# leerob/pixo

Measured on NVIDIA H100. Metric: Mpixels/sec JPEG q=80 4:2:0 encode of 3840x2160 RGB, higher is better.
Workload: dtype f32

## Files before the change

### pixo_b200/csrc/api.cu

```cuda
#include <stdarg.h>
#include <stdlib.h>
#include <string.h>

#include <emmintrin.h>

#include <algorithm>
#include <cmath>
#include <thread>
#include <vector>

#include "common.cuh"
#include "jpeg_host.hpp"
#include "resize_host.hpp"

namespace pixo {

static thread_local std::string g_thread_err;

int set_error(pixo_b200_ctx *ctx, int code, const char *fmt, ...)
{
    char buf[512];
    va_list ap;
    va_start(ap, fmt);
    vsnprintf(buf, sizeof buf, fmt, ap);
// ... 404 lines not shown
    const uint8_t *vals[4];
    for (int k = 0; k < 4; ++k) {
        memcpy(bits[k], dht + k * 272, 16);
        vals[k] = dht + k * 272 + 16;
    }
    if (!prog_tables(bits, vals, T))
        return set_error(ctx, PIXO_B200_ERR_INVALID_ARGUMENT,
                         "Huffman table: more than 256 values, or a code that does not fit its length");
    return 0;
}

static int check_room(pixo_b200_ctx *ctx, size_t out_cap, size_t need)
{
    if (need > out_cap)
        return set_error(ctx, PIXO_B200_ERR_OUTPUT_TOO_SMALL, "output capacity %zu too small (need %zu)", out_cap, need);
    return 0;
}

static int finish_frame(pixo_b200_ctx *ctx, uint8_t *out, size_t out_cap, size_t hdr, size_t body, size_t *out_len)
{
    if (body == (size_t)-1)
        return set_error(ctx, PIXO_B200_ERR_OUTPUT_TOO_SMALL, "output capacity %zu too small", out_cap);
    PIXO_TRY(check_room(ctx, out_cap, hdr + body + 2));
    out[hdr + body] = 0xFF;
    out[hdr + body + 1] = 0xD9;
    *out_len = hdr + body + 2;
    return 0;
}

struct CoefLayout {
    size_t yb, cbb, yeb, ceb, each;
    explicit CoefLayout(const FrameGeometry &g)
        : yb(Layout::round(g.ny * 64 * sizeof(int16_t))), cbb(Layout::round(g.nc * 64 * sizeof(int16_t))),
          yeb(Layout::round(g.ny)), ceb(Layout::round(g.nc)), each(yb + 2 * cbb + yeb + 2 * ceb) {}
    size_t stride() const { return each / sizeof(int16_t); }
    int16_t *y(void *frame) const { return reinterpret_cast<int16_t *>(frame); }
    int16_t *cb(void *frame) const { return reinterpret_cast<int16_t *>(static_cast<uint8_t *>(frame) + yb); }
    int16_t *cr(void *frame) const { return reinterpret_cast<int16_t *>(static_cast<uint8_t *>(frame) + yb + cbb); }
    CoefExtents extents(void *frame) const
    {
        uint8_t *e = static_cast<uint8_t *>(frame) + yb + 2 * cbb;
        return CoefExtents{e, e + yeb, e + yeb + ceb, each};
    }
};

static void expand_records(const CoefLayout &L, const FrameGeometry &g, void *frame)
{
    const CoefExtents e = L.extents(frame);
    int16_t *arr[3] = {L.y(frame), L.cb(frame), L.cr(frame)};
    const uint8_t *ext[3] = {e.y, e.cb, e.cr};
    const size_t nb[3] = {g.ny, g.nc, g.nc};
    for (int c = 0; c < (g.has_chroma ? 3 : 1); ++c)
        for (size_t b = 0; b < nb[c]; ++b) {
            const int sectors = ext[c][b];
            memset(arr[c] + b * 64 + sectors * 16, 0, (size_t)(4 - sectors) * 32);
        }
}

void pixo_b200_quant_tables(int quality, uint8_t lum_zz[64], uint8_t chr_zz[64], float lum[64],
                            float chr[64])
{
    quant_tables(quality, lum_zz, chr_zz, lum, chr);
}

int pixo_b200_jpeg_block_counts(uint32_t width, uint32_t height, uint32_t color_type,
                                uint32_t subsampling, size_t *ny, size_t *nc)
{
    PIXO_TRY(validate_jpeg(nullptr, width, height, color_type, subsampling));
    const FrameGeometry g = make_geometry(width, height, color_type, subsampling);
    if (ny) *ny = g.ny;
    if (nc) *nc = g.nc;
    return 0;
}

static int trellis_status(pixo_b200_ctx *ctx, const uint32_t *d_status)
{
    PIXO_TRY(ctx->h_trellis.ensure(ctx, sizeof(uint32_t)));
    PIXO_CUDA(ctx, cudaMemcpyAsync(ctx->h_trellis.ptr, d_status, sizeof(uint32_t), cudaMemcpyDeviceToHost, ctx->stream));
    PIXO_CUDA(ctx, cudaStreamSynchronize(ctx->stream));
    if (*static_cast<const uint32_t *>(ctx->h_trellis.ptr))
        return set_error(ctx, PIXO_B200_ERR_INVALID_ARGUMENT,
                         "trellis input out of range: a non-finite value or cost, a non-zero |dct| below 2^-100, or |dct / q| above 32766");
    return 0;
}

static constexpr size_t kTrellisScratch = (size_t)256 << 20;

static int trellis_pieces(pixo_b200_ctx *ctx, const uint8_t *d_pixels, size_t pixel_stride, uint32_t n_images,
// ... 1478 lines not shown
```

### pixo_b200/csrc/common.cuh

```cuda
#pragma once

#include <cuda_runtime.h>
#include <stdint.h>
#include <stdio.h>

#include <atomic>
#include <condition_variable>
#include <functional>
#include <memory>
#include <mutex>
#include <string>
#include <thread>
#include <unordered_map>
#include <utility>
#include <vector>

#include "../../include/pixo_b200.h"

namespace pixo {

constexpr int kHistWords = 536;
constexpr size_t kDhtBytes = 4 * 272;
constexpr size_t kHuffDevBytes = 1632;

__host__ __device__ constexpr int zz_nat(int i)
{
    constexpr int t[64] = {0,  1,  8,  16, 9,  2,  3,  10, 17, 24, 32, 25, 18, 11, 4,  5,
                           12, 19, 26, 33, 40, 48, 41, 34, 27, 20, 13, 6,  7,  14, 21, 28,
                           35, 42, 49, 56, 57, 50, 43, 36, 29, 22, 15, 23, 30, 37, 44, 51,
                           58, 59, 52, 45, 38, 31, 39, 46, 53, 60, 61, 54, 47, 55, 62, 63};
    return t[i];
}

struct CoefExtents {
    uint8_t *y, *cb, *cr;
    size_t stride;
};

constexpr uint32_t kOvfNoFit = 1u;
constexpr uint32_t kOvfFault = 2u;
constexpr uint32_t kOvfSegment = 4u;
constexpr uint32_t kOvfRange = 8u;
constexpr uint32_t kOvfInput = 16u;

template <bool Pinned>
struct Buffer {
    void *ptr = nullptr;
    size_t cap = 0;
    Buffer() = default;
    Buffer(const Buffer &) = delete;
    Buffer &operator=(const Buffer &) = delete;
    ~Buffer()
    {
        if (ptr) Pinned ? cudaFreeHost(ptr) : cudaFree(ptr);
    }
    int ensure(pixo_b200_ctx *ctx, size_t bytes);
    uint8_t *slot(size_t i, size_t stride) const { return static_cast<uint8_t *>(ptr) + i * stride; }
};
using DevBuf = Buffer<false>;
using PinnedBuf = Buffer<true>;

class HostPool {
public:
    explicit HostPool(int nthreads);
    ~HostPool();
    void run(int njobs, const std::function<void(int)> &fn);

private:
    void worker();
    std::vector<std::thread> threads_;
// ... 233 lines not shown
```

### pixo_b200/csrc/jpeg_entropy.cu

```cuda
#include <type_traits>

#include "common.cuh"
#include "jpeg_host.hpp"

namespace pixo {
namespace {

constexpr int AC_STRIDE = 12, AC_ZRL = 190, AC_EOB = 191, AC_WORDS = 192;
struct HuffDev {
    uint32_t dc[2][12];
    uint32_t ac[2][AC_WORDS];
};
static_assert(sizeof(HuffDev) == kHuffDevBytes, "common.cuh sizes the per-frame tables by kHuffDevBytes");
struct HuffHalf {
    uint32_t dc[12];
    uint32_t ac[AC_WORDS];
};
struct FrameTables {
    const HuffDev *tabs;
};

struct EntParams {
    const int16_t *y, *cb, *cr;
    size_t y_stride, c_stride;
// ... 327 lines not shown
        uint32_t srel[NPASS], t7[NPASS];
#pragma unroll 1
        for (int p = 0; p < NPASS; ++p) {
            uint32_t mm, kk, comp;
            if (ypm == 4) {
                if (p < 2) { mm = 8 * p + (lane >> 2); kk = lane & 3; comp = 0; }
                else { mm = lane & 15; kk = 4 + (lane >> 4); comp = 1 + (lane >> 4); }
            } else if (bpm == 3) {
                mm = lane; kk = p; comp = p;
            } else {
                mm = 32 * p + lane; kk = 0; comp = 0;
            }
            const uint32_t sr = mm * bpm + kk;
            const bool valid = sr < nv;
            uint32_t *const slot = M.slot[p];
            uint32_t L = 0, tail7 = 0;
            int nwt = 0;
            if (__any_sync(0xffffffffu, valid)) {
                if constexpr (TABLES) {
                    const uint32_t half = comp ? 1u : 0u;
                    const uint32_t key = ((RAW && P.seg_per_img > 1) ? C.img / P.seg_per_img : C.img) * 2u + half;
                    if (key != tab_key) {
                        const uint32_t *src = reinterpret_cast<const uint32_t *>(Tp.tabs + (key >> 1));
                        uint32_t *dst = reinterpret_cast<uint32_t *>(&T[threadIdx.x >> 5]);
                        __syncwarp();
                        for (int i = lane; i < 12 + AC_WORDS; i += 32)
                            dst[i] = __ldg(src + (i < 12 ? half * 12 + i : 24 + half * AC_WORDS + (i - 12)));
                        __syncwarp();
                        tab_key = key;
                    }
                }
                const uint32_t m = mu0 + mm;
                const int16_t *arr;
                const uint8_t *earr;
                size_t idx, eidx;
                int seed;
                if (comp == 0) { arr = P.y + y_off; earr = P.e.y; idx = (size_t)m * ypm + kk; eidx = ey_off + idx; seed = P.dc_seed[0]; }
                else if (comp == 1) { arr = P.cb + c_off; earr = P.e.cb; idx = m; eidx = ec_off + idx; seed = P.dc_seed[1]; }
                else { arr = P.cr + c_off; earr = P.e.cr; idx = m; eidx = ec_off + idx; seed = P.dc_seed[2]; }
                const bool from_left = lane != 0 && !(ypm == 4 && p == 2 && lane == 16);
                int prev_ld = 0;
                if (valid && !from_left) {
                    const bool dc_reset = P.rst_mcus && C.first && mm == 0;
                    if (P.dc_seed_dev && idx == 0 && !seg_prev) seed = P.dc_seed_dev[comp];
                    prev_ld = dc_reset ? 0 : ((idx || seg_prev) ? arr[((long long)idx - 1) * 64] : seed);
                }
                int dc = 0;
                uint32_t M0 = 0, M1 = 0;
                if (valid) {
                    const uint4 *src = reinterpret_cast<const uint4 *>(arr + idx * 64);
                    uint32_t w[32];
                    if (CHECK) {
                        uint32_t n[32];
#pragma unroll
                        for (int q = 0; q < 8; ++q) {
                            const uint4 v = __ldg(src + q);
                            n[q * 4] = v.x; n[q * 4 + 1] = v.y; n[q * 4 + 2] = v.z; n[q * 4 + 3] = v.w;
                        }
                        dc = (int)(int16_t)(n[0] & 0xFFFF);
#pragma unroll
                        for (int j = 0; j < 32; ++j) {
                            const int i0 = zz_nat(2 * j), i1 = zz_nat(2 * j + 1);
                            w[j] = __byte_perm(n[i0 >> 1], n[i1 >> 1],
                                               ((i0 & 1) ? 0x0032 : 0x0010) | ((i1 & 1) ? 0x7600 : 0x5400));
                        }
#pragma unroll
                        for (int j = 0; j < 32; ++j) M.stage[j * CB + lane] = w[j];
                    } else {
                        const int np = 2 * __ldg(earr + eidx);
#pragma unroll
                        for (int q = 0; q < 8; ++q) {
                            const uint4 v = (q < 2 || q < np) ? __ldg(src + q) : make_uint4(0, 0, 0, 0);
                            w[q * 4] = v.x; w[q * 4 + 1] = v.y; w[q * 4 + 2] = v.z; w[q * 4 + 3] = v.w;
                        }
                        dc = (int)(int16_t)(w[0] & 0xFFFF);
#pragma unroll
                        for (int q = 0; q < 8; ++q) {
                            if (q < 2 || q < np) {
#pragma unroll
                                for (int t = 0; t < 4; ++t) M.stage[(q * 4 + t) * CB + lane] = w[q * 4 + t];
                            }
                        }
                    }
                    asm volatile("" ::: "memory");
                    {
                        uint32_t e0 = 0, e1 = 0;
#pragma unroll
                        for (int j = 0; j < 16; ++j) {
                            e0 += __vminu2(w[j], 0x00010001u) * (1u << j);
                            e1 += __vminu2(w[16 + j], 0x00010001u) * (1u << j);
                        }
                        M0 = interleave16(e0); M1 = interleave16(e1);
                    }
                }
                const int left = __shfl_up_sync(0xffffffffu, dc, 1);
                const int diff = (int)(int16_t)(dc - (from_left ? left : prev_ld));
                if (valid) {
                    const int tbl = comp ? 1 : 0;
                    const uint32_t *dctab;
                    uint32_t sa_ac;
                    if constexpr (TABLES) {
                        dctab = T[threadIdx.x >> 5].dc;
                        sa_ac = (uint32_t)__cvta_generic_to_shared(&T[threadIdx.x >> 5].ac[0]);
                    } else {
                        dctab = T.dc[tbl];
                        sa_ac = (uint32_t)__cvta_generic_to_shared(&T.ac[tbl][0]);
                    }
                    const uint32_t sa_slot = (uint32_t)__cvta_generic_to_shared(slot) + 4u * lane;
                    uint32_t acc;
                    bool bad;
                    L = code_block<false, CHECK>(M0, M1, diff, dctab, sa_ac, sa_stage, sa_slot, spill[p], &acc, &bad);
                    if (L > SLOT_W * 32u)
                        L = code_block<true, CHECK>(M0, M1, diff, dctab, sa_ac, sa_stage, sa_slot, spill[p], &acc, &bad);
                    if (CHECK && bad) atomicOr(&P.overflow[C.img], kOvfRange);
                    asm volatile("" ::: "memory");
                    const int nw = (int)(L >> 5), filled = (int)(L & 31u);
                    nwt = nw;
                    if (filled) {
                        if (nw < SLOT_W) slot[nw * CB + lane] = acc; else spill[p][nw - SLOT_W] = acc;
                        nwt = nw + 1;
                    }
                    const uint32_t lastw = nw == 0 ? 0u : (nw - 1 < SLOT_W ? slot[(nw - 1) * CB + lane] : spill[p][nw - 1 - SLOT_W]);
                    tail7 = __funnelshift_rc(acc, lastw, 32 - filled) & 0x7Fu;
                }
            }
// ... 1129 lines not shown
```

### pixo_b200/csrc/jpeg_transform.cu

```cuda
#include <cuda.h>
#include <string.h>

#include <algorithm>

#include "common.cuh"

namespace pixo {
namespace {

#define FADD(a, b) __fadd_rn((a), (b))
#define FSUB(a, b) __fsub_rn((a), (b))
#define FMUL(a, b) __fmul_rn((a), (b))

#define AAN_A1 0.70710678118654752440f
#define AAN_A2 0.5411961f
#define AAN_A3 0.70710678118654752440f
#define AAN_A4 1.3065629f
#define AAN_A5 0.38268343f
#define AAN_S0 0.3535534f
#define AAN_S1 0.2548978f
#define AAN_S2 0.2705981f
#define AAN_S3 0.3006724f
#define AAN_S4 0.3535534f
#define AAN_S5 0.4499881f
// ... 177 lines not shown
}

struct __align__(16) QPair {
    float nd_lo, nd_hi, r_lo, r_hi;
};

struct QPairTab {
    QPair t[2][32];
};


__device__ __forceinline__ void dct_rows_x2(f2 (&R)[4][8], f2 (&C)[8][4])
{
    constexpr float SK[8] = {AAN_S0, AAN_S1, AAN_S2, AAN_S3, AAN_S4, AAN_S5, AAN_S6, AAN_S7};
#pragma unroll
    for (int i = 0; i < 4; ++i) {
        f2 o[8];
        aan_1d_x2_core(R[i], o);
#pragma unroll
        for (int j = 0; j < 4; ++j) {
            float a0, a1, b0, b1;
            mulc(o[2 * j], SK[2 * j], a0, a1);
            mulc(o[2 * j + 1], SK[2 * j + 1], b0, b1);
            C[2 * i][j] = pk(a0, b0);
            C[2 * i + 1][j] = pk(a1, b1);
        }
    }
}

enum CoefOut { kNatural, kZigzag, kRecords, kDct };

template <int OUT, typename TabFn>
__device__ __forceinline__ void dct_cols_quant_store_x2(f2 (&C)[8][4], TabFn tab, uint4 *__restrict__ out,
                                                        const int swz, uint8_t *eout, float *dout, float dscale)
{
    constexpr bool ZIGZAG = OUT != kNatural;
    constexpr float SK[8] = {AAN_S0, AAN_S1, AAN_S2, AAN_S3, AAN_S4, AAN_S5, AAN_S6, AAN_S7};
    if constexpr (OUT == kDct) {
#pragma unroll
        for (int j = 0; j < 4; ++j) {
            const f2 in[8] = {C[0][j], C[1][j], C[2][j], C[3][j], C[4][j], C[5][j], C[6][j], C[7][j]};
            f2 o[8];
            aan_1d_x2_core(in, o);
#pragma unroll
            for (int r = 0; r < 8; ++r) {
                const f2 x = mul2(mul2(o[r], K2(SK[r])), K2(dscale));
                if (dout) *reinterpret_cast<float2 *>(dout + r * 8 + 2 * j) = make_float2(x.lo, x.hi);
            }
        }
        return;
    }
    uint32_t W[32];
    const f2 half2 = K2(0.5f), magic2 = K2(12582912.0f);
    uint32_t kSign, kOne;
    asm("mov.b32 %0, 0x80000000;" : "=r"(kSign));
    asm("mov.b32 %0, 0x3F800000;" : "=r"(kOne));
#pragma unroll
    for (int j = 0; j < 4; ++j) {
        QPair T[8];
#pragma unroll
        for (int r = 0; r < 8; ++r) T[r] = tab(r * 4 + j);
        const f2 in[8] = {C[0][j], C[1][j], C[2][j], C[3][j], C[4][j], C[5][j], C[6][j], C[7][j]};
        f2 o[8];
        aan_1d_x2_core(in, o);
#pragma unroll
        for (int r = 0; r < 8; ++r) {
            const f2 nd = pk(T[r].nd_lo, T[r].nd_hi), rc = pk(T[r].r_lo, T[r].r_hi);
// ... 1 lines not shown
            const f2 q0 = mul2(x, rc);
            const f2 e = fma2(q0, nd, x);
            const f2 q = fma2(e, rc, q0);
            uint32_t ql, qh;
            upk_u(q, ql, qh);
            uint32_t sl, sh;
            asm("lop3.b32 %0, %1, %2, %3, 0xEA;" : "=r"(sl) : "r"(ql), "r"(kSign), "r"(kOne));
            asm("lop3.b32 %0, %1, %2, %3, 0xEA;" : "=r"(sh) : "r"(qh), "r"(kSign), "r"(kOne));
            const f2 sg = pk(__uint_as_float(sl), __uint_as_float(sh));
            const f2 w = add2_rz(q, half2);
            const f2 tt = fma2_rm(w, sg, magic2);
            uint32_t tl, th, neg;
            upk_u(tt, tl, th);
            asm("prmt.b32 %0, %1, %2, %3;" : "=r"(neg) : "r"(ql), "r"(qh), "r"(0xFFBBu));
            W[r * 4 + j] = __byte_perm(tl, th, 0x5410) ^ neg;
        }
    }
    uint32_t Z[32];
#pragma unroll
    for (int k = 0; k < 8; ++k) {
#pragma unroll
        for (int m = 0; m < 4; ++m) {
            if (ZIGZAG) {
                const int i0 = zz_nat(k * 8 + m * 2), i1 = zz_nat(k * 8 + m * 2 + 1);
                Z[k * 4 + m] = __byte_perm(W[i0 >> 1], W[i1 >> 1],
                                           ((i0 & 1) ? 0x0032 : 0x0010) | ((i1 & 1) ? 0x7600 : 0x5400));
            } else {
                Z[k * 4 + m] = W[k * 4 + m];
            }
        }
        out[k ^ swz] = make_uint4(Z[k * 4], Z[k * 4 + 1], Z[k * 4 + 2], Z[k * 4 + 3]);
    }
    if (OUT == kRecords) {
        uint32_t o[4] = {0, 0, 0, 0};
#pragma unroll
        for (int i = 8; i < 32; ++i) o[i >> 3] |= Z[i];
        *eout = (uint8_t)(o[3] ? 4 : o[2] ? 3 : o[1] ? 2 : 1);
    }
}

template <int OUT>
__device__ __forceinline__ void dct_quant_store_x2(f2 (&R)[4][8], const QPairTab *qs, const bool chroma_u,
                                                   uint4 *__restrict__ out, const int swz, uint8_t *eout,
                                                   float *dout = nullptr, float dscale = 1.0f)
{
    f2 C[8][4];
    dct_rows_x2(R, C);
    const QPair *t = qs->t[chroma_u ? 1 : 0];
    dct_cols_quant_store_x2<OUT>(C, [&](int i) { return t[i]; }, out, swz, eout, dout, dscale);
}

template <int OUT, typename SwzFn, typename DstFn, typename EDstFn>
__device__ __forceinline__ void flush_stage(const uint4 *__restrict__ stage, const uint8_t *ext, int lane,
                                            SwzFn swz_of, DstFn dst_of, EDstFn edst_of)
{
    __syncwarp();
    uint32_t e[8];
    if (OUT == kRecords) {
        const uint4 a = reinterpret_cast<const uint4 *>(ext)[0], b = reinterpret_cast<const uint4 *>(ext)[1];
        e[0] = a.x; e[1] = a.y; e[2] = a.z; e[3] = a.w; e[4] = b.x; e[5] = b.y; e[6] = b.z; e[7] = b.w;
    }
#pragma unroll
    for (int j = 0; j < 8; ++j) {
        const int s = j * 4 + (lane >> 3), k = lane & 7;
        const uint4 v = stage[s * 8 + (k ^ swz_of(s))];
        uint4 *d = dst_of(s);
        if (OUT != kRecords) {
            if (d) d[k] = v;
        } else {
            const uint32_t keep = (d != nullptr) & ((uint32_t)(k >> 1) < __byte_perm(e[j], 0, 0x4440 + (lane >> 3)));
            asm volatile("{\n\t.reg .pred p;\n\tsetp.ne.u32 p, %5, 0;\n\t"
                         "@p st.global.v4.u32 [%0], {%1, %2, %3, %4};\n\t}"
                         :: "l"(d + k), "r"(v.x), "r"(v.y), "r"(v.z), "r"(v.w), "r"(keep) : "memory");
        }
    }
    if (OUT == kRecords) {
        uint8_t *ed = edst_of(lane);
        if (ed) *ed = ext[lane];
    }
    __syncwarp();
}

__device__ __forceinline__ uint32_t smem_u32(const void *p)
{
    return (uint32_t)__cvta_generic_to_shared(p);
}
__device__ __forceinline__ void mbar_init(uint64_t *bar, uint32_t count)
{
    asm volatile("mbarrier.init.shared::cta.b64 [%0], %1;" ::"r"(smem_u32(bar)), "r"(count));
}
__device__ __forceinline__ void mbar_expect_tx(uint64_t *bar, uint32_t bytes)
{
    asm volatile("mbarrier.arrive.expect_tx.shared::cta.b64 _, [%0], %1;" ::"r"(smem_u32(bar)),
                 "r"(bytes)
                 : "memory");
}
__device__ __forceinline__ void mbar_wait(uint64_t *bar, uint32_t parity)
{
    asm volatile(
        "{\n\t.reg .pred p;\n\t"
        "WAIT_%=:\n\t"
        "mbarrier.try_wait.parity.shared::cta.b64 p, [%0], %1;\n\t"
        "@p bra DONE_%=;\n\t"
        "bra WAIT_%=;\n\t"
        "DONE_%=:\n\t}" ::"r"(smem_u32(bar)),
        "r"(parity)
        : "memory");
}
__device__ __forceinline__ void tma_load_3d(void *dst, const void *tmap, int x, int y, int z,
                                            uint64_t *bar)
{
    asm volatile(
        "cp.async.bulk.tensor.3d.shared::cluster.global.mbarrier::complete_tx::bytes "
        "[%0], [%1, {%2, %3, %4}], [%5];" ::"r"(smem_u32(dst)),
        "l"(tmap), "r"(x), "r"(y), "r"(z), "r"(smem_u32(bar))
        : "memory");
}

constexpr int K1_WARPS = 4;
constexpr int K1_THREADS = K1_WARPS * 32;
constexpr int K1_MIN_BLOCKS = 2;
constexpr int K1_MCUS = 16;
constexpr int K1_HB = 8 * 16 * 3;
constexpr int K1_HALF_BYTES = 16 * K1_HB;
constexpr int K1_TILE_BYTES = 2 * K1_HALF_BYTES;

struct K1Params {
    const uint8_t *pixels;
    size_t pixel_stride;
    uint32_t w, h, mcus_x, mcus_y, units_x, n_images;
    int16_t *y, *cb, *cr;
    size_t y_stride, c_stride;
    CoefExtents e;
    uint32_t use_tma;
};

struct __align__(128) K1WarpSmem {
    uint8_t tile[2][K1_HALF_BYTES];
    uint32_t csum[K1_MCUS * 64];
    __align__(16) uint8_t ext[32];
    uint64_t bar;
};

struct __align__(128) K1Smem {
    K1WarpSmem w[K1_WARPS];
    QPairTab q;
};

__device__ __forceinline__ void rgb_windows8(const uint32_t (&w)[6], uint32_t (&win)[8])
{
    win[0] = w[0];
    win[1] = __funnelshift_r(w[0], w[1], 24);
    win[2] = __funnelshift_r(w[1], w[2], 16);
    win[3] = w[2] >> 8;
    win[4] = w[3];
    win[5] = __funnelshift_r(w[3], w[4], 24);
    win[6] = __funnelshift_r(w[4], w[5], 16);
    win[7] = w[5] >> 8;
}

__device__ __forceinline__ void ycc_row8(const uint32_t (&w)[6], float (&yv)[8], uint32_t (&hs)[4])
{
    uint32_t win[8];
    rgb_windows8(w, win);
    uint32_t pp[8];
#pragma unroll
    for (int x = 0; x < 8; ++x) {
        const uint32_t ys = __dp4a(win[x], 0x001D964Du, 128u);
        const int ucb = dp4a_us(win[x], 0x0080552Bu, -32641);
        const int ucr = dp4a_us(win[x], 0x00156B80u, -32641);
        yv[x] = __uint_as_float(__byte_perm(ys, 0x4B000000u, 0x7651));
        pp[x] = __vmaxu2(__byte_perm((uint32_t)ucb, (uint32_t)ucr, 0x7531), 0xFF01FF01u);
    }
// ... 145 lines not shown
                            v0[hh * 4 + k] = __uint_as_float(__byte_perm(a[k], 0x4B000000u, sel));
                            v1[hh * 4 + k] = __uint_as_float(__byte_perm(b[k], 0x4B000000u, sel));
                        }
                    }
#pragma unroll
                    for (int x = 0; x < 8; ++x) R[i][x] = sub2(K2(bias), pk(v0[x], v1[x]));
                }
                __syncwarp();
                stage = reinterpret_cast<uint4 *>(WS.csum);
                slot = lane;
                swz = slot & 7;
            }
            if constexpr (OUT == kDct) {
                float *dout = nullptr;
                if (!chroma_u) {
                    if (job * 8u + (slot >> 2) < n_mcu)
                        dout = reinterpret_cast<float *>(P.y) + (size_t)img * P.y_stride + ((mcu_base + job * 8) * 4 + slot) * 64;
                } else if ((uint32_t)(lane & 15) < n_mcu) {
                    dout = reinterpret_cast<float *>(lane < 16 ? P.cb : P.cr) + (size_t)img * P.c_stride +
                           (mcu_base + (lane & 15)) * 64;
                }
                dct_quant_store_x2<OUT>(R, QS, chroma_u, stage + slot * 8, swz, &WS.ext[slot], dout,
                                        chroma_u ? 0.25f : 1.0f);
                continue;
            }
            dct_quant_store_x2<OUT>(R, QS, chroma_u, stage + slot * 8, swz, &WS.ext[slot]);
            if (!chroma_u) {
                const size_t b0 = (mcu_base + job * 8) * 4;
                uint4 *ybase = reinterpret_cast<uint4 *>(P.y + (size_t)img * P.y_stride + b0 * 64);
                const uint32_t first = job * 8;
                flush_stage<OUT>(
                    stage, WS.ext, lane, [](int s) { return ((s >> 3) << 1) | (s & 1); },
                    [&](int s) -> uint4 * { return first + (s >> 2) < n_mcu ? ybase + s * 8 : nullptr; },
                    [&](int s) -> uint8_t * {
                        return first + (s >> 2) < n_mcu ? P.e.y + ((size_t)img * P.e.stride + b0 + s) : nullptr;
                    });
            } else {
                uint4 *cbb = reinterpret_cast<uint4 *>(P.cb + (size_t)img * P.c_stride + mcu_base * 64);
                uint4 *crb = reinterpret_cast<uint4 *>(P.cr + (size_t)img * P.c_stride + mcu_base * 64);
                flush_stage<OUT>(
                    stage, WS.ext, lane, [](int s) { return s & 7; },
                    [&](int s) -> uint4 * {
                        return (uint32_t)(s & 15) < n_mcu ? (s < 16 ? cbb : crb) + (s & 15) * 8 : nullptr;
                    },
                    [&](int s) -> uint8_t * {
                        return (uint32_t)(s & 15) < n_mcu
                                   ? (s < 16 ? P.e.cb : P.e.cr) + ((size_t)img * P.e.stride + mcu_base + (s & 15))
                                   : nullptr;
                    });
            }
        }
        img = img_n; my = my_n; ux = ux_n;
    }
}

constexpr int GRAY_BLOCKS = 64;

__device__ __forceinline__ void y_row8(const uint32_t (&w)[6], float (&v)[8])
{
    uint32_t win[8];
    rgb_windows8(w, win);
#pragma unroll
    for (int x = 0; x < 8; ++x)
        v[x] = byte1_to_float_minus(__dp4a(win[x], 0x001D964Du, 128u), 8388736.0f);
}
__device__ __forceinline__ void c_row8(const uint32_t (&w)[6], uint32_t wgt, float (&v)[8])
{
    uint32_t win[8];
    rgb_windows8(w, win);
#pragma unroll
    for (int x = 0; x < 8; ++x) {
        const int u = max(dp4a_us(win[x], wgt, -32641), -65280);
        v[x] = FSUB(8388736.0f, __uint_as_float(__byte_perm((uint32_t)u, 0x4B000000u, 0x7651)));
    }
}

constexpr int K444_WARPS = 4;
constexpr int K444_THREADS = K444_WARPS * 32;
constexpr int K444_ROW_B = 32 * 8 * 3;
constexpr int K444_TILE_BYTES = 8 * K444_ROW_B;
constexpr int K444_MIN_BLOCKS = 2;

struct __align__(128) K444WarpSmem {
    uint8_t tile[2][K444_TILE_BYTES];
    uint4 stage[256];
    __align__(16) uint8_t ext[32];
    uint64_t bar[2];
};

struct __align__(128) K444Smem {
    K444WarpSmem w[K444_WARPS];
    QPairTab q;
};

template <int OUT>
__global__ void __launch_bounds__(K444_THREADS, K444_MIN_BLOCKS)
k_jpeg_444(const __grid_constant__ K1Params P, const __grid_constant__ QPairTab qp,
           const __grid_constant__ CUtensorMap tmap)
{
    extern __shared__ __align__(128) uint8_t smem_raw[];
    K444Smem &S = *reinterpret_cast<K444Smem *>(smem_raw);
    const int tid = threadIdx.x, lane = tid & 31, warp = tid >> 5;
    K444WarpSmem &WS = S.w[warp];
    for (int i = tid; i < 64; i += K444_THREADS) S.q.t[i >> 5][i & 31] = qp.t[i >> 5][i & 31];
    const QPairTab *QS = &S.q;
    if (lane == 0) {
        mbar_init(&WS.bar[0], 1);
        mbar_init(&WS.bar[1], 1);
        asm volatile("fence.mbarrier_init.release.cluster;" ::: "memory");
    }
    __syncthreads();

    const uint32_t units_per_img = P.mcus_y * P.units_x;
    const uint64_t nunits = (uint64_t)units_per_img * P.n_images;
    const uint32_t stride = gridDim.x * K444_WARPS;
    const uint32_t d_ux = stride % P.units_x, d_t = stride / P.units_x;
    const uint32_t d_by = d_t % P.mcus_y, d_img = d_t / P.mcus_y;
    uint32_t phase = 0;

// ... 14 lines not shown
    };

    uint64_t u = (uint64_t)blockIdx.x * K444_WARPS + warp;
    uint32_t img, by, ux;
    {
        const uint32_t u0 = blockIdx.x * K444_WARPS + warp;
        img = u0 / units_per_img;
        const uint32_t rem = u0 - img * units_per_img;
        by = rem / P.units_x;
        ux = rem - by * P.units_x;
    }
    int b = 0;
    if (u < nunits && lane == 0) issue_tma(img, by, ux, 0);
    for (; u < nunits; u += stride, b ^= 1) {
        uint32_t img_n = img, by_n = by, ux_n = ux;
        advance(img_n, by_n, ux_n);
        if (lane == 0 && u + stride < nunits) issue_tma(img_n, by_n, ux_n, b ^ 1);
        if (unit_by_tma(by)) {
            mbar_wait(&WS.bar[b], (phase >> b) & 1u);
            phase ^= 1u << b;
        } else {
            const uint8_t *image = P.pixels + (size_t)img * P.pixel_stride;
            warp_load_tile_rgb<8, 256>(WS.tile[b], image, P.w, P.h, ux * 256, by * 8, lane);
            __syncwarp();
        }
        const uint32_t bx0 = ux * 32;
        const uint8_t *base = WS.tile[b] + lane * 24;
        auto row_words = [&](int r, uint32_t (&wds)[6]) {
            const uint2 *p = reinterpret_cast<const uint2 *>(base + r * K444_ROW_B);
            const uint2 a = p[0], c1 = p[1], c2 = p[2];
            wds[0] = a.x; wds[1] = a.y; wds[2] = c1.x; wds[3] = c1.y; wds[4] = c2.x; wds[5] = c2.y;
        };
        const size_t b0 = (size_t)by * P.mcus_x + bx0;
        auto flush = [&](int16_t *arr, uint8_t *earr) {
            uint4 *dbase = reinterpret_cast<uint4 *>(arr + b0 * 64);
            flush_stage<OUT>(
                WS.stage, WS.ext, lane, [](int s) { return s & 7; },
                [&](int s) -> uint4 * { return bx0 + s < P.mcus_x ? dbase + s * 8 : nullptr; },
                [&](int s) -> uint8_t * { return bx0 + s < P.mcus_x ? earr + s : nullptr; });
        };
#pragma unroll 1
        for (int comp = 0; comp < 3; ++comp) {
            const bool chroma_u = __ballot_sync(0xffffffffu, comp != 0) != 0u;
            f2 R[4][8];
            if (!chroma_u) {
#pragma unroll
                for (int rp = 0; rp < 4; ++rp) {
                    float v0[8], v1[8];
                    uint32_t wa[6], wb[6];
                    row_words(rp * 2, wa); row_words(rp * 2 + 1, wb);
                    y_row8(wa, v0); y_row8(wb, v1);
#pragma unroll
                    for (int x = 0; x < 8; ++x) R[rp][x] = pk(v0[x], v1[x]);
                }
            } else {
                const uint32_t wgt = comp == 1 ? 0x0080552Bu : 0x00156B80u;
#pragma unroll
                for (int rp = 0; rp < 4; ++rp) {
                    float v0[8], v1[8];
                    uint32_t wa[6], wb[6];
                    row_words(rp * 2, wa); row_words(rp * 2 + 1, wb);
                    c_row8(wa, wgt, v0); c_row8(wb, wgt, v1);
#pragma unroll
                    for (int x = 0; x < 8; ++x) R[rp][x] = pk(v0[x], v1[x]);
                }
            }
            if constexpr (OUT == kDct) {
                float *arr = reinterpret_cast<float *>(comp == 0 ? P.y : (comp == 1 ? P.cb : P.cr)) +
                             (size_t)img * (comp == 0 ? P.y_stride : P.c_stride);
                dct_quant_store_x2<OUT>(R, QS, chroma_u, WS.stage + lane * 8, lane & 7, &WS.ext[lane],
                                        bx0 + lane < P.mcus_x ? arr + (b0 + lane) * 64 : nullptr);
                continue;
            }
            dct_quant_store_x2<OUT>(R, QS, chroma_u, WS.stage + lane * 8, lane & 7, &WS.ext[lane]);
            uint8_t *earr = nullptr;
            if (OUT == kRecords)
                earr = (comp == 0 ? P.e.y : (comp == 1 ? P.e.cb : P.e.cr)) + ((size_t)img * P.e.stride + b0);
            flush(comp == 0 ? P.y + (size_t)img * P.y_stride : (comp == 1 ? P.cb : P.cr) + (size_t)img * P.c_stride, earr);
        }
        __syncwarp();
        img = img_n; by = by_n; ux = ux_n;
    }
}

template <int OUT>
__global__ void __launch_bounds__(64)
k_jpeg_gray(const uint8_t *__restrict__ pixels, size_t pixel_stride, uint32_t w, uint32_t h,
            uint32_t blocks_x, uint32_t tiles_x, int16_t *__restrict__ yout, size_t y_stride,
            uint8_t *__restrict__ yext, size_t e_stride, const __grid_constant__ QPairTab qp)
{
    constexpr int TB = GRAY_BLOCKS * 8;
    __shared__ __align__(16) uint8_t tile[8 * TB];
    __shared__ __align__(16) uint4 stage[2][256];
    __shared__ __align__(16) uint8_t ext[2][32];
    __shared__ QPairTab qsm;
    for (int i = threadIdx.x; i < 64; i += 64) qsm.t[i >> 5][i & 31] = qp.t[i >> 5][i & 31];
    const QPairTab *QS = &qsm;
    const int tid = threadIdx.x, lane = tid & 31, warp = tid >> 5;
    const uint32_t tx = blockIdx.x % tiles_x;
    const uint32_t brow = blockIdx.x / tiles_x;
    const uint32_t img = blockIdx.y;
    const uint8_t *image = pixels + (size_t)img * pixel_stride;
    load_tile<1, 8, GRAY_BLOCKS * 8, 64>(tile, image, w, h, tx * (GRAY_BLOCKS * 8), brow * 8, tid);
    __syncthreads();
    const int j = tid;
    const uint32_t b0 = tx * GRAY_BLOCKS;
    {
        f2 R[4][8];
#pragma unroll
        for (int rp = 0; rp < 4; ++rp) {
            const uint2 a = *reinterpret_cast<const uint2 *>(tile + (rp * 2) * TB + j * 8);
            const uint2 b = *reinterpret_cast<const uint2 *>(tile + (rp * 2 + 1) * TB + j * 8);
            const uint32_t wa[2] = {a.x, a.y}, wb[2] = {b.x, b.y};
#pragma unroll
            for (int x = 0; x < 8; ++x) {
                const float f0 = __uint_as_float(__byte_perm(wa[x >> 2], 0x4B000000u, 0x7650 + (x & 3)));
                const float f1 = __uint_as_float(__byte_perm(wb[x >> 2], 0x4B000000u, 0x7650 + (x & 3)));
                R[rp][x] = sub2(pk(f0, f1), K2(8388736.0f));
            }
        }
        if constexpr (OUT == kDct) {
            const uint32_t blk = b0 + j;
            dct_quant_store_x2<OUT>(R, QS, false, stage[warp] + lane * 8, lane & 7, &ext[warp][lane],
                                    blk < blocks_x ? reinterpret_cast<float *>(yout) + (size_t)img * y_stride +
                                                         ((size_t)brow * blocks_x + blk) * 64
                                                   : nullptr);
            return;
        }
        dct_quant_store_x2<OUT>(R, QS, false, stage[warp] + lane * 8, lane & 7, &ext[warp][lane]);
    }
    const uint32_t first = b0 + warp * 32;
    const size_t bfirst = (size_t)brow * blocks_x + first;
    uint4 *dbase = reinterpret_cast<uint4 *>(yout + (size_t)img * y_stride + bfirst * 64);
    flush_stage<OUT>(
        stage[warp], ext[warp], lane, [](int s) { return s & 7; },
        [&](int s) -> uint4 * { return first + s < blocks_x ? dbase + s * 8 : nullptr; },
        [&](int s) -> uint8_t * {
            return first + s < blocks_x ? yext + ((size_t)img * e_stride + bfirst + s) : nullptr;
        });
}

__device__ __forceinline__ int category16(int v)
{
    const int a = v < 0 ? -v : v;
    return 32 - __clz(a);
}

template <int IN>
__global__ void __launch_bounds__(256)
k_jpeg_hist(const int16_t *__restrict__ ycoef, size_t y_stride, const int16_t *__restrict__ cbcoef,
            const int16_t *__restrict__ crcoef, size_t c_stride, const CoefExtents E, size_t ny, size_t nc,
            uint32_t blocks_y_per_mcu, uint32_t restart_interval,
            unsigned long long *__restrict__ hist, const int seed_y, const int seed_cb, const int seed_cr)
{
    __shared__ uint32_t sh[kHistWords];
    for (int i = threadIdx.x; i < kHistWords; i += blockDim.x) sh[i] = 0;
    __syncthreads();
    const uint32_t img = blockIdx.y;
    const size_t total = ny + 2 * nc;
    for (size_t b = (size_t)blockIdx.x * blockDim.x + threadIdx.x; b < total;
         b += (size_t)gridDim.x * blockDim.x) {
        const int16_t *arr;
        const uint8_t *earr;
        size_t idx;
        bool lum;
        uint32_t per_mcu;
        int seed;
        if (b < ny) { arr = ycoef + (size_t)img * y_stride; earr = E.y; idx = b; lum = true; per_mcu = blocks_y_per_mcu; seed = seed_y; }
        else if (b < ny + nc) { arr = cbcoef + (size_t)img * c_stride; earr = E.cb; idx = b - ny; lum = false; per_mcu = 1; seed = seed_cb; }
        else { arr = crcoef + (size_t)img * c_stride; earr = E.cr; idx = b - ny - nc; lum = false; per_mcu = 1; seed = seed_cr; }
        const uint4 *src = reinterpret_cast<const uint4 *>(arr + idx * 64);
        const int np = IN == kRecords ? 2 * __ldg(earr + ((size_t)img * E.stride + idx)) : 8;
        uint32_t wv[32];
#pragma unroll
        for (int k = 0; k < 8; ++k) {
            const uint4 t = k < np ? __ldg(src + k) : make_uint4(0, 0, 0, 0);
            wv[k * 4] = t.x; wv[k * 4 + 1] = t.y; wv[k * 4 + 2] = t.z; wv[k * 4 + 3] = t.w;
        }
        const size_t mcu = idx / per_mcu;
        const bool first_in_mcu = (idx % per_mcu) == 0;
        const bool reset = restart_interval && first_in_mcu && (mcu % restart_interval) == 0;
        const int prev = reset ? 0 : (idx ? (int)arr[(idx - 1) * 64] : seed);
        const int dc = (int)(int16_t)(wv[0] & 0xFFFF);
        const int diff = (int)(int16_t)(dc - prev);
        atomicAdd(&sh[(lum ? 0 : 12) + min(category16(diff), 11)], 1u);
        uint32_t *ac = sh + (lum ? 24 : 280);
        int run = 0;
#pragma unroll
        for (int i = 1; i < 64; ++i) {
            const int nat = IN != kNatural ? i : zz_nat(i);
            const uint32_t word = wv[nat >> 1];
            const int c = (int)(int16_t)((nat & 1) ? (word >> 16) : (word & 0xFFFF));
            if (c == 0) {
                ++run;
            } else {
                if (run >= 16) { atomicAdd(&ac[0xF0], (uint32_t)(run >> 4)); run &= 15; }
                atomicAdd(&ac[(run << 4) | min(category16(c), 10)], 1u);
                run = 0;
            }
        }
        if (run > 0) atomicAdd(&ac[0], 1u);
    }
    __syncthreads();
    for (int i = threadIdx.x; i < kHistWords; i += blockDim.x)
        if (sh[i]) atomicAdd(&hist[(size_t)img * kHistWords + i], (unsigned long long)sh[i]);
}

void fill_qpair_tab(const float *lum_q, const float *chr_q, float chr_scale, QPairTab *qp)
{
    for (int c = 0; c < 2; ++c) {
        const float *d = c ? chr_q : lum_q;
        const float sc = c ? chr_scale : 1.0f;
        for (int w = 0; w < 32; ++w) {
            volatile float r0 = 1.0f / d[2 * w], r1 = 1.0f / d[2 * w + 1];
            QPair e;
            e.nd_lo = -(d[2 * w] * sc);
// ... 86 lines not shown
}

int transform(pixo_b200_ctx *ctx, const uint8_t *d_pixels, size_t pixel_stride, uint32_t n_images, uint32_t w,
              uint32_t h, uint32_t color_type, uint32_t subsampling, const float *lum_q, const float *chr_q,
              int out, void *d_y_, size_t y_stride, void *d_cb_, void *d_cr_, size_t c_stride, const CoefExtents *ext)
{
    QPairTab qt;
    fill_qpair_tab(lum_q, chr_q, (color_type != PIXO_B200_GRAY && subsampling == PIXO_B200_S420) ? 4.0f : 1.0f, &qt);
    const size_t esz = out == kDct ? sizeof(float) : sizeof(int16_t);
    auto at = [esz](void *base, size_t elems) -> int16_t * {
        return base ? reinterpret_cast<int16_t *>(static_cast<uint8_t *>(base) + elems * esz) : nullptr;
    };
    for (int i = 0; i < 64; ++i) {
        const float a = lum_q[i], b = chr_q[i];
        if (!(a >= 1.0f && a <= 255.0f && a == (float)(int)a && b >= 1.0f && b <= 255.0f &&
              b == (float)(int)b))
            return set_error(ctx, PIXO_B200_ERR_INVALID_ARGUMENT,
                             "quantisation table entries must be integers in 1..255");
    }
    const uint64_t units_max = (uint64_t)((w + 7) / 8 + 31) / 32 * ((h + 7) / 8);
    const uint32_t per_launch = (uint32_t)std::min<uint64_t>(65535, 0xFFFFFFFFull / (units_max ? units_max : 1));
    for (uint32_t i0 = 0; i0 < n_images; i0 += per_launch) {
        const uint32_t nb = n_images - i0 < per_launch ? n_images - i0 : per_launch;
        const uint8_t *px = d_pixels + (size_t)i0 * pixel_stride;
        int16_t *y = at(d_y_, (size_t)i0 * y_stride);
        int16_t *cb = at(d_cb_, (size_t)i0 * c_stride);
        int16_t *cr = at(d_cr_, (size_t)i0 * c_stride);
        const CoefExtents e = extents_from(ext, i0);
        if (color_type == PIXO_B200_GRAY) {
            const uint32_t bx = (w + 7) / 8, by = (h + 7) / 8;
            const uint32_t tiles_x = (bx + GRAY_BLOCKS - 1) / GRAY_BLOCKS;
            dim3 grid(tiles_x * by, nb);
            void (*const kg[4])(const uint8_t *, size_t, uint32_t, uint32_t, uint32_t, uint32_t, int16_t *, size_t,
                                uint8_t *, size_t, QPairTab) = {k_jpeg_gray<kNatural>, k_jpeg_gray<kZigzag>,
                                                                 k_jpeg_gray<kRecords>, k_jpeg_gray<kDct>};
            PIXO_TRY(launch(ctx, kg[out], grid, 64, 0, px, pixel_stride, w, h, bx, tiles_x, y, y_stride, e.y, e.stride, qt));
        } else {
            PIXO_TRY(launch_rgb_transform(ctx, subsampling == PIXO_B200_S444, out, px, pixel_stride, nb, w, h, y,
                                          y_stride, cb, cr, c_stride, e, qt));
        }
    }
    return 0;
}

}

int launch_jpeg_transform(pixo_b200_ctx *ctx, const uint8_t *d_pixels, size_t pixel_stride,
                          uint32_t n_images, uint32_t w, uint32_t h, uint32_t color_type,
                          uint32_t subsampling, const float *lum_q, const float *chr_q,
                          int16_t *d_y, size_t y_stride, int16_t *d_cb, int16_t *d_cr,
                          size_t c_stride, uint32_t flags, const CoefExtents *ext)
{
    const int out = ext ? kRecords : (flags & PIXO_B200_COEF_ZIGZAG) ? kZigzag : kNatural;
    return transform(ctx, d_pixels, pixel_stride, n_images, w, h, color_type, subsampling, lum_q, chr_q, out, d_y,
                     y_stride, d_cb, d_cr, c_stride, ext);
}

int launch_jpeg_transform_dct(pixo_b200_ctx *ctx, const uint8_t *d_pixels, size_t pixel_stride, uint32_t n_images,
                              uint32_t w, uint32_t h, uint32_t color_type, uint32_t subsampling,
                              const float *lum_q, const float *chr_q, float *d_y, size_t y_stride, float *d_cb,
                              float *d_cr, size_t c_stride)
{
    return transform(ctx, d_pixels, pixel_stride, n_images, w, h, color_type, subsampling, lum_q, chr_q, kDct, d_y,
                     y_stride, d_cb, d_cr, c_stride, nullptr);
}

int launch_jpeg_histogram(pixo_b200_ctx *ctx, const int16_t *d_y, size_t y_stride,
// ... 33 lines not shown
```

Before: 221,100.

## Pack DC value and sector count into 32-bit per-block side records

Widens each block's extent byte to a 32-bit side word holding the quantised DC coefficient and the count of nonzero 16-coefficient sectors, which can now be zero. The transform kernels write this word. The entropy and histogram kernels read DC and the previous block's DC from it instead of reloading coefficient rows, and skip storing and loading the first two uint4s of all-zero-AC blocks. This cuts scattered global reads of neighbouring blocks' DC values and the writes of empty sectors, but quadruples the side-array size and adds a host fixup that writes DC back into the expanded coefficients.

```diff
diff --git a/pixo_b200/csrc/api.cu b/pixo_b200/csrc/api.cu
--- a/pixo_b200/csrc/api.cu
+++ b/pixo_b200/csrc/api.cu
@@ -460,7 +460,8 @@
     size_t yb, cbb, yeb, ceb, each;
     explicit CoefLayout(const FrameGeometry &g)
         : yb(Layout::round(g.ny * 64 * sizeof(int16_t))), cbb(Layout::round(g.nc * 64 * sizeof(int16_t))),
-          yeb(Layout::round(g.ny)), ceb(Layout::round(g.nc)), each(yb + 2 * cbb + yeb + 2 * ceb) {}
+          yeb(Layout::round(g.ny * sizeof(uint32_t))), ceb(Layout::round(g.nc * sizeof(uint32_t))),
+          each(yb + 2 * cbb + yeb + 2 * ceb) {}
     size_t stride() const { return each / sizeof(int16_t); }
     int16_t *y(void *frame) const { return reinterpret_cast<int16_t *>(frame); }
     int16_t *cb(void *frame) const { return reinterpret_cast<int16_t *>(static_cast<uint8_t *>(frame) + yb); }
@@ -468,7 +469,8 @@
     CoefExtents extents(void *frame) const
     {
         uint8_t *e = static_cast<uint8_t *>(frame) + yb + 2 * cbb;
-        return CoefExtents{e, e + yeb, e + yeb + ceb, each};
+        return CoefExtents{reinterpret_cast<uint32_t *>(e), reinterpret_cast<uint32_t *>(e + yeb),
+                           reinterpret_cast<uint32_t *>(e + yeb + ceb), each / sizeof(uint32_t)};
     }
 };
 
@@ -476,12 +478,14 @@
 {
     const CoefExtents e = L.extents(frame);
     int16_t *arr[3] = {L.y(frame), L.cb(frame), L.cr(frame)};
-    const uint8_t *ext[3] = {e.y, e.cb, e.cr};
+    const uint32_t *side[3] = {e.y, e.cb, e.cr};
     const size_t nb[3] = {g.ny, g.nc, g.nc};
     for (int c = 0; c < (g.has_chroma ? 3 : 1); ++c)
         for (size_t b = 0; b < nb[c]; ++b) {
-            const int sectors = ext[c][b];
-            memset(arr[c] + b * 64 + sectors * 16, 0, (size_t)(4 - sectors) * 32);
+            int16_t *blk = arr[c] + b * 64;
+            const int sectors = side_sectors(side[c][b]);
+            memset(blk + sectors * 16, 0, (size_t)(4 - sectors) * 32);
+            blk[0] = (int16_t)side_dc(side[c][b]);
         }
 }
 
diff --git a/pixo_b200/csrc/common.cuh b/pixo_b200/csrc/common.cuh
--- a/pixo_b200/csrc/common.cuh
+++ b/pixo_b200/csrc/common.cuh
@@ -33,9 +33,11 @@
 }
 
 struct CoefExtents {
-    uint8_t *y, *cb, *cr;
+    uint32_t *y, *cb, *cr;
     size_t stride;
 };
+__host__ __device__ inline int side_dc(uint32_t s) { return (int)(int16_t)(s & 0xFFFFu); }
+__host__ __device__ inline int side_sectors(uint32_t s) { return (int)((s >> 16) & 7u); }
 
 constexpr uint32_t kOvfNoFit = 1u;
 constexpr uint32_t kOvfFault = 2u;
diff --git a/pixo_b200/csrc/jpeg_entropy.cu b/pixo_b200/csrc/jpeg_entropy.cu
--- a/pixo_b200/csrc/jpeg_entropy.cu
+++ b/pixo_b200/csrc/jpeg_entropy.cu
@@ -383,7 +383,7 @@
                 }
                 const uint32_t m = mu0 + mm;
                 const int16_t *arr;
-                const uint8_t *earr;
+                const uint32_t *earr;
                 size_t idx, eidx;
                 int seed;
                 if (comp == 0) { arr = P.y + y_off; earr = P.e.y; idx = (size_t)m * ypm + kk; eidx = ey_off + idx; seed = P.dc_seed[0]; }
@@ -394,13 +394,16 @@
                 if (valid && !from_left) {
                     const bool dc_reset = P.rst_mcus && C.first && mm == 0;
                     if (P.dc_seed_dev && idx == 0 && !seg_prev) seed = P.dc_seed_dev[comp];
-                    prev_ld = dc_reset ? 0 : ((idx || seg_prev) ? arr[((long long)idx - 1) * 64] : seed);
+                    prev_ld = dc_reset ? 0
+                            : !(idx || seg_prev) ? seed
+                            : CHECK ? arr[((long long)idx - 1) * 64] : side_dc(__ldg(earr + (eidx - 1)));
                 }
                 int dc = 0;
                 uint32_t M0 = 0, M1 = 0;
                 if (valid) {
                     const uint4 *src = reinterpret_cast<const uint4 *>(arr + idx * 64);
                     uint32_t w[32];
+                    uint32_t side = 0;
                     if (CHECK) {
                         uint32_t n[32];
 #pragma unroll
@@ -418,16 +421,17 @@
 #pragma unroll
                         for (int j = 0; j < 32; ++j) M.stage[j * CB + lane] = w[j];
                     } else {
-                        const int np = 2 * __ldg(earr + eidx);
+                        side = __ldg(earr + eidx);
+                        const int np = 2 * side_sectors(side);
 #pragma unroll
                         for (int q = 0; q < 8; ++q) {
                             const uint4 v = (q < 2 || q < np) ? __ldg(src + q) : make_uint4(0, 0, 0, 0);
                             w[q * 4] = v.x; w[q * 4 + 1] = v.y; w[q * 4 + 2] = v.z; w[q * 4 + 3] = v.w;
                         }
-                        dc = (int)(int16_t)(w[0] & 0xFFFF);
+                        dc = side_dc(side);
 #pragma unroll
                         for (int q = 0; q < 8; ++q) {
-                            if (q < 2 || q < np) {
+                            if (q < np) {
 #pragma unroll
                                 for (int t = 0; t < 4; ++t) M.stage[(q * 4 + t) * CB + lane] = w[q * 4 + t];
                             }
@@ -442,6 +446,7 @@
                             e1 += __vminu2(w[16 + j], 0x00010001u) * (1u << j);
                         }
                         M0 = interleave16(e0); M1 = interleave16(e1);
+                        if (!CHECK && side_sectors(side) == 0) M0 = M1 = 0u;
                     }
                 }
                 const int left = __shfl_up_sync(0xffffffffu, dc, 1);
diff --git a/pixo_b200/csrc/jpeg_transform.cu b/pixo_b200/csrc/jpeg_transform.cu
--- a/pixo_b200/csrc/jpeg_transform.cu
+++ b/pixo_b200/csrc/jpeg_transform.cu
@@ -233,7 +233,7 @@
 
 template <int OUT, typename TabFn>
 __device__ __forceinline__ void dct_cols_quant_store_x2(f2 (&C)[8][4], TabFn tab, uint4 *__restrict__ out,
-                                                        const int swz, uint8_t *eout, float *dout, float dscale)
+                                                        const int swz, uint32_t *eout, float *dout, float dscale)
 {
     constexpr bool ZIGZAG = OUT != kNatural;
     constexpr float SK[8] = {AAN_S0, AAN_S1, AAN_S2, AAN_S3, AAN_S4, AAN_S5, AAN_S6, AAN_S7};
@@ -301,16 +301,16 @@
         out[k ^ swz] = make_uint4(Z[k * 4], Z[k * 4 + 1], Z[k * 4 + 2], Z[k * 4 + 3]);
     }
     if (OUT == kRecords) {
-        uint32_t o[4] = {0, 0, 0, 0};
-#pragma unroll
-        for (int i = 8; i < 32; ++i) o[i >> 3] |= Z[i];
-        *eout = (uint8_t)(o[3] ? 4 : o[2] ? 3 : o[1] ? 2 : 1);
+        uint32_t o[4] = {Z[0] & 0xFFFF0000u, 0, 0, 0};
+#pragma unroll
+        for (int i = 1; i < 32; ++i) o[i >> 3] |= Z[i];
+        *eout = (Z[0] & 0xFFFFu) | ((o[3] ? 4u : o[2] ? 3u : o[1] ? 2u : o[0] ? 1u : 0u) << 16);
     }
 }
 
 template <int OUT>
 __device__ __forceinline__ void dct_quant_store_x2(f2 (&R)[4][8], const QPairTab *qs, const bool chroma_u,
-                                                   uint4 *__restrict__ out, const int swz, uint8_t *eout,
+                                                   uint4 *__restrict__ out, const int swz, uint32_t *eout,
                                                    float *dout = nullptr, float dscale = 1.0f)
 {
     f2 C[8][4];
@@ -320,15 +320,10 @@
 }
 
 template <int OUT, typename SwzFn, typename DstFn, typename EDstFn>
-__device__ __forceinline__ void flush_stage(const uint4 *__restrict__ stage, const uint8_t *ext, int lane,
+__device__ __forceinline__ void flush_stage(const uint4 *__restrict__ stage, const uint32_t *ext, int lane,
                                             SwzFn swz_of, DstFn dst_of, EDstFn edst_of)
 {
     __syncwarp();
-    uint32_t e[8];
-    if (OUT == kRecords) {
-        const uint4 a = reinterpret_cast<const uint4 *>(ext)[0], b = reinterpret_cast<const uint4 *>(ext)[1];
-        e[0] = a.x; e[1] = a.y; e[2] = a.z; e[3] = a.w; e[4] = b.x; e[5] = b.y; e[6] = b.z; e[7] = b.w;
-    }
 #pragma unroll
     for (int j = 0; j < 8; ++j) {
         const int s = j * 4 + (lane >> 3), k = lane & 7;
@@ -337,14 +332,14 @@
         if (OUT != kRecords) {
             if (d) d[k] = v;
         } else {
-            const uint32_t keep = (d != nullptr) & ((uint32_t)(k >> 1) < __byte_perm(e[j], 0, 0x4440 + (lane >> 3)));
+            const uint32_t keep = (d != nullptr) & ((k >> 1) < side_sectors(ext[s]));
             asm volatile("{\n\t.reg .pred p;\n\tsetp.ne.u32 p, %5, 0;\n\t"
                          "@p st.global.v4.u32 [%0], {%1, %2, %3, %4};\n\t}"
                          :: "l"(d + k), "r"(v.x), "r"(v.y), "r"(v.z), "r"(v.w), "r"(keep) : "memory");
         }
     }
     if (OUT == kRecords) {
-        uint8_t *ed = edst_of(lane);
+        uint32_t *ed = edst_of(lane);
         if (ed) *ed = ext[lane];
     }
     __syncwarp();
@@ -407,7 +402,7 @@
 struct __align__(128) K1WarpSmem {
     uint8_t tile[2][K1_HALF_BYTES];
     uint32_t csum[K1_MCUS * 64];
-    __align__(16) uint8_t ext[32];
+    uint32_t ext[32];
     uint64_t bar;
 };
 
@@ -619,7 +614,7 @@
                 flush_stage<OUT>(
                     stage, WS.ext, lane, [](int s) { return ((s >> 3) << 1) | (s & 1); },
                     [&](int s) -> uint4 * { return first + (s >> 2) < n_mcu ? ybase + s * 8 : nullptr; },
-                    [&](int s) -> uint8_t * {
+                    [&](int s) -> uint32_t * {
                         return first + (s >> 2) < n_mcu ? P.e.y + ((size_t)img * P.e.stride + b0 + s) : nullptr;
                     });
             } else {
@@ -630,7 +625,7 @@
                     [&](int s) -> uint4 * {
                         return (uint32_t)(s & 15) < n_mcu ? (s < 16 ? cbb : crb) + (s & 15) * 8 : nullptr;
                     },
-                    [&](int s) -> uint8_t * {
+                    [&](int s) -> uint32_t * {
                         return (uint32_t)(s & 15) < n_mcu
                                    ? (s < 16 ? P.e.cb : P.e.cr) + ((size_t)img * P.e.stride + mcu_base + (s & 15))
                                    : nullptr;
@@ -671,7 +666,7 @@
 struct __align__(128) K444WarpSmem {
     uint8_t tile[2][K444_TILE_BYTES];
     uint4 stage[256];
-    __align__(16) uint8_t ext[32];
+    uint32_t ext[32];
     uint64_t bar[2];
 };
 
@@ -752,12 +747,12 @@
             wds[0] = a.x; wds[1] = a.y; wds[2] = c1.x; wds[3] = c1.y; wds[4] = c2.x; wds[5] = c2.y;
         };
         const size_t b0 = (size_t)by * P.mcus_x + bx0;
-        auto flush = [&](int16_t *arr, uint8_t *earr) {
+        auto flush = [&](int16_t *arr, uint32_t *earr) {
             uint4 *dbase = reinterpret_cast<uint4 *>(arr + b0 * 64);
             flush_stage<OUT>(
                 WS.stage, WS.ext, lane, [](int s) { return s & 7; },
                 [&](int s) -> uint4 * { return bx0 + s < P.mcus_x ? dbase + s * 8 : nullptr; },
-                [&](int s) -> uint8_t * { return bx0 + s < P.mcus_x ? earr + s : nullptr; });
+                [&](int s) -> uint32_t * { return bx0 + s < P.mcus_x ? earr + s : nullptr; });
         };
 #pragma unroll 1
         for (int comp = 0; comp < 3; ++comp) {
@@ -793,7 +788,7 @@
                 continue;
             }
             dct_quant_store_x2<OUT>(R, QS, chroma_u, WS.stage + lane * 8, lane & 7, &WS.ext[lane]);
-            uint8_t *earr = nullptr;
+            uint32_t *earr = nullptr;
             if (OUT == kRecords)
                 earr = (comp == 0 ? P.e.y : (comp == 1 ? P.e.cb : P.e.cr)) + ((size_t)img * P.e.stride + b0);
             flush(comp == 0 ? P.y + (size_t)img * P.y_stride : (comp == 1 ? P.cb : P.cr) + (size_t)img * P.c_stride, earr);
@@ -807,12 +802,12 @@
 __global__ void __launch_bounds__(64)
 k_jpeg_gray(const uint8_t *__restrict__ pixels, size_t pixel_stride, uint32_t w, uint32_t h,
             uint32_t blocks_x, uint32_t tiles_x, int16_t *__restrict__ yout, size_t y_stride,
-            uint8_t *__restrict__ yext, size_t e_stride, const __grid_constant__ QPairTab qp)
+            uint32_t *__restrict__ yext, size_t e_stride, const __grid_constant__ QPairTab qp)
 {
     constexpr int TB = GRAY_BLOCKS * 8;
     __shared__ __align__(16) uint8_t tile[8 * TB];
     __shared__ __align__(16) uint4 stage[2][256];
-    __shared__ __align__(16) uint8_t ext[2][32];
+    __shared__ uint32_t ext[2][32];
     __shared__ QPairTab qsm;
     for (int i = threadIdx.x; i < 64; i += 64) qsm.t[i >> 5][i & 31] = qp.t[i >> 5][i & 31];
     const QPairTab *QS = &qsm;
@@ -855,7 +850,7 @@
     flush_stage<OUT>(
         stage[warp], ext[warp], lane, [](int s) { return s & 7; },
         [&](int s) -> uint4 * { return first + s < blocks_x ? dbase + s * 8 : nullptr; },
-        [&](int s) -> uint8_t * {
+        [&](int s) -> uint32_t * {
             return first + s < blocks_x ? yext + ((size_t)img * e_stride + bfirst + s) : nullptr;
         });
 }
@@ -881,7 +876,7 @@
     for (size_t b = (size_t)blockIdx.x * blockDim.x + threadIdx.x; b < total;
          b += (size_t)gridDim.x * blockDim.x) {
         const int16_t *arr;
-        const uint8_t *earr;
+        const uint32_t *earr;
         size_t idx;
         bool lum;
         uint32_t per_mcu;
@@ -890,7 +885,8 @@
         else if (b < ny + nc) { arr = cbcoef + (size_t)img * c_stride; earr = E.cb; idx = b - ny; lum = false; per_mcu = 1; seed = seed_cb; }
         else { arr = crcoef + (size_t)img * c_stride; earr = E.cr; idx = b - ny - nc; lum = false; per_mcu = 1; seed = seed_cr; }
         const uint4 *src = reinterpret_cast<const uint4 *>(arr + idx * 64);
-        const int np = IN == kRecords ? 2 * __ldg(earr + ((size_t)img * E.stride + idx)) : 8;
+        const uint32_t *side = IN == kRecords ? earr + ((size_t)img * E.stride + idx) : nullptr;
+        const int np = IN == kRecords ? 2 * side_sectors(__ldg(side)) : 8;
         uint32_t wv[32];
 #pragma unroll
         for (int k = 0; k < 8; ++k) {
@@ -900,8 +896,8 @@
         const size_t mcu = idx / per_mcu;
         const bool first_in_mcu = (idx % per_mcu) == 0;
         const bool reset = restart_interval && first_in_mcu && (mcu % restart_interval) == 0;
-        const int prev = reset ? 0 : (idx ? (int)arr[(idx - 1) * 64] : seed);
-        const int dc = (int)(int16_t)(wv[0] & 0xFFFF);
+        const int prev = reset ? 0 : !idx ? seed : IN == kRecords ? side_dc(__ldg(side - 1)) : (int)arr[(idx - 1) * 64];
+        const int dc = IN == kRecords ? side_dc(__ldg(side)) : (int)(int16_t)(wv[0] & 0xFFFF);
         const int diff = (int)(int16_t)(dc - prev);
         atomicAdd(&sh[(lum ? 0 : 12) + min(category16(diff), 11)], 1u);
         uint32_t *ac = sh + (lum ? 24 : 280);
@@ -1054,7 +1050,7 @@
             const uint32_t tiles_x = (bx + GRAY_BLOCKS - 1) / GRAY_BLOCKS;
             dim3 grid(tiles_x * by, nb);
             void (*const kg[4])(const uint8_t *, size_t, uint32_t, uint32_t, uint32_t, uint32_t, int16_t *, size_t,
-                                uint8_t *, size_t, QPairTab) = {k_jpeg_gray<kNatural>, k_jpeg_gray<kZigzag>,
+                                uint32_t *, size_t, QPairTab) = {k_jpeg_gray<kNatural>, k_jpeg_gray<kZigzag>,
                                                                  k_jpeg_gray<kRecords>, k_jpeg_gray<kDct>};
             PIXO_TRY(launch(ctx, kg[out], grid, 64, 0, px, pixel_stride, w, h, bx, tiles_x, y, y_stride, e.y, e.stride, qt));
         } else {
```

Result: no change. 222,700 (median of 6 runs) (+0.7%).
